# alxfox/AR_Voxel_Project

Hardware: AMD Instinct MI355X
Metric: Mvoxel-views/s (voxels x views / s) + carve wall-time, 512^3 grid x 36 views (higher is better)
Workload: dtype u8; 1 GPU; synthetic sphere silhouettes, 512x512x512 grid, 36 views 640x480, per step: derive bit planes + summed-area tables from the resident u8 masks, then dense carve of a fresh model by all views; one step after the other; views=36, jobs_in_flight=1, parallelism=single GPU, collective=none, cull=True

## Files before the change

### ar_voxel_project_amd/capi.py

```python
from __future__ import annotations

import ctypes as C
import os
from typing import Optional, Sequence, Tuple

import numpy as np

_HERE = os.path.dirname(os.path.abspath(__file__))
LIB_PATH = os.environ.get("ARVX_LIB_PATH") or os.path.join(_HERE, "lib", "libarvx.so")

OCC = 1
SEEN = 2
CARVE_NO_CULL = 1
CARVE_STATS = 2
CARVE_FUSED = 8
CARVE_STREAM = 16
CARVE_FILTER = 64
CARVE_NO_STREAM = 32
CARVE_DENSE_CLASSIFY = 128
CARVE_WHOLE_ITEMS = 256
PATH_DENSE_CLASSIFY = 1
PATH_ITEM_SHARING = 2
PATH_FRESH = 4
PATH_LAZY_CODES = 8
PATH_FUSED = 16
PATH_BRUTE_FORCE = 32
PATH_STREAM = 64
FLOOD_PREPASS = 1
FLOOD_FRESH = 2
VOTES_COUNTS = 1
VOTES_NO_CULL = 2
COMPONENTS_LARGEST = 1
_EXTRA_CARVE_FLAGS = int(os.environ.get("ARVX_CARVE_EXTRA_FLAGS", "0"))
COLOR_CLOSEST = 0
COLOR_AVERAGE = 1

SYMBOLS = [
    "arvx_version", "arvx_last_error", "arvx_device_count", "arvx_projection_assoc",
    "arvx_ctx_create_slab_halo",
    "arvx_set_projection_assoc", "arvx_ctx_set_projection_assoc", "arvx_ctx_projection_assoc",
    "arvx_selftest_project", "arvx_selftest_depth", "arvx_selftest_view_tables",
    "arvx_ctx_create", "arvx_ctx_create_slab", "arvx_ctx_create_striped", "arvx_ctx_destroy",
    "arvx_ctx_set_stream", "arvx_ctx_set_exchange_stream", "arvx_ctx_synchronize", "arvx_ctx_voxels",
    "arvx_compose_projection", "arvx_set_views", "arvx_set_views_device",
    "arvx_set_images", "arvx_state_reset", "arvx_state_upload",
    "arvx_state_download", "arvx_state_device_ptr", "arvx_state_upload_halo",
    "arvx_state_upload_planes", "arvx_state_download_planes", "arvx_state_packet_geometry",
    "arvx_state_download_packets", "arvx_host_register",
    "arvx_host_unregister", "arvx_handle_unseen", "arvx_undistort", "arvx_undistort_device",
    "arvx_pack_occupancy", "arvx_pack_occupancy_global", "arvx_carve", "arvx_carve_views", "arvx_fast_carve",
    "arvx_color", "arvx_surface_count", "arvx_surface_download",
    "arvx_surface_depth_download", "arvx_color_samples",
    "arvx_color_visible", "arvx_surface_visible_download", "arvx_view_depth_download",
    "arvx_photo_carve", "arvx_carve_votes", "arvx_votes_download",
    "arvx_components", "arvx_components_download", "arvx_components_labels_download",
    "arvx_components_keep",
    "arvx_colors_upload", "arvx_closure", "arvx_closure_count", "arvx_closure_download",
    "arvx_closure_download32",
    "arvx_mc_cells", "arvx_mc_cells_download", "arvx_mc_mesh", "arvx_mc_mesh_download",
    "arvx_mc_mesh_download_faces", "arvx_mc_mesh_welded", "arvx_mc_mesh_welded_download",
    "arvx_mc_mesh_smooth", "arvx_mc_mesh_smooth_download",
    "arvx_render", "arvx_render_view", "arvx_render_download", "arvx_render_agreement",
    "arvx_occupancy_packet_words", "arvx_occupancy_compress", "arvx_occupancy_expand",
    "arvx_occupancy_expand_striped", "arvx_occupancy_pack_compress", "arvx_occupancy_expand_striped_others",
    "arvx_export_model", "arvx_get_stats", "arvx_last_carve_path", "arvx_last_fast_carve_path",
    "arvx_selftest_divide",
    "arvx_selftest_round",
]


class ArvxError(RuntimeError):
    def __init__(self, code: int, msg: str):
        super().__init__(f"arvx error {code}: {msg}")
        self.code = code


class Stats(C.Structure):
    _fields_ = [
        ("subtiles", C.c_uint64),
        ("subtiles_carved", C.c_uint64),
        ("subtile_views_mixed", C.c_uint64),
        ("subtile_views_total", C.c_uint64),
        ("surface_voxels", C.c_uint64),
        ("reserved", C.c_uint64 * 3),
        ("host_total_fallbacks", C.c_uint64),
    ]


_libs: dict = {}
ASSOC_RIGHT, ASSOC_LEFT = 0, 1
# ... 55 lines not shown
    lib.arvx_pack_occupancy_global.argtypes = [p, p]
    lib.arvx_carve.argtypes = [p, C.c_uint]
    lib.arvx_carve_views.argtypes = [p, C.c_int, C.c_int, C.c_uint]
    lib.arvx_fast_carve.argtypes = [p]
    lib.arvx_color.argtypes = [p, C.c_int]
    lib.arvx_surface_count.argtypes = [p, C.POINTER(C.c_int64)]
    lib.arvx_surface_download.argtypes = [p, C.POINTER(C.c_int64), f32p]
    lib.arvx_surface_depth_download.argtypes = [p, f32p]
    lib.arvx_colors_upload.argtypes = [p, C.c_int64, C.POINTER(C.c_int64), f32p]
    lib.arvx_closure.argtypes = [p, C.c_int, C.c_int]
    lib.arvx_closure_count.argtypes = [p, C.POINTER(C.c_int64)]
    lib.arvx_closure_download.argtypes = [p, C.POINTER(C.c_int64), f32p]
    lib.arvx_export_model.argtypes = [p, f32p, C.c_int]
    lib.arvx_get_stats.argtypes = [p, C.POINTER(Stats)]
    if hasattr(lib, "arvx_last_carve_path"):
        lib.arvx_last_carve_path.argtypes = [p, C.POINTER(C.c_uint32)]
    if hasattr(lib, "arvx_last_fast_carve_path"):
        lib.arvx_last_fast_carve_path.argtypes = [p, C.POINTER(C.c_uint32)]
    ab_build = bool(os.environ.get("ARVX_LIB_PATH"))
    if hasattr(lib, "arvx_selftest_divide") or not ab_build:
        lib.arvx_selftest_divide.argtypes = [p, C.c_int64, f32p, f32p, f32p, f32p]
    if hasattr(lib, "arvx_selftest_round") or not ab_build:
        lib.arvx_selftest_round.argtypes = [p, C.POINTER(C.c_int64)]
    if hasattr(lib, "arvx_mc_cells") or not ab_build:
        lib.arvx_mc_cells.argtypes = [p, C.POINTER(C.c_int64)]
        lib.arvx_mc_cells_download.argtypes = [p, C.POINTER(C.c_int32)]
    if hasattr(lib, "arvx_occupancy_compress") or not ab_build:
        lib.arvx_occupancy_packet_words.argtypes = [C.c_int64, C.c_int64]
        lib.arvx_occupancy_compress.argtypes = [p, C.c_void_p, C.c_int64, C.c_void_p, C.c_int64]
        lib.arvx_occupancy_expand.argtypes = [p, C.c_void_p, C.c_int, C.c_int, C.c_int64,
                                              C.c_int64, C.c_void_p, C.c_void_p]
        if hasattr(lib, "arvx_occupancy_expand_striped") or not ab_build:
            lib.arvx_occupancy_expand_striped.argtypes = [p, C.c_void_p, C.c_int, C.c_int64,
                                                          C.c_int64, C.c_int64, C.c_void_p,
                                                          C.c_void_p]
        if hasattr(lib, "arvx_occupancy_pack_compress"):
            lib.arvx_occupancy_pack_compress.argtypes = [p, C.c_void_p, C.c_int64, C.c_void_p]
            lib.arvx_occupancy_expand_striped_others.argtypes = [p, C.c_void_p, C.c_int, C.c_int, C.c_int64,
                                                                 C.c_int64, C.c_int64, C.c_void_p, C.c_void_p]
    if hasattr(lib, "arvx_mc_mesh_smooth"):
        lib.arvx_mc_mesh_smooth.argtypes = [p, C.c_int, C.c_float, C.c_float]
        lib.arvx_mc_mesh_smooth_download.argtypes = [p, C.c_void_p, C.c_void_p]
    if hasattr(lib, "arvx_color_visible"):
        lib.arvx_color_visible.argtypes = [p, C.c_int, C.c_float]
        lib.arvx_surface_visible_download.argtypes = [p, C.POINTER(C.c_int32)]
        lib.arvx_view_depth_download.argtypes = [p, C.c_int, f32p]
# ... 576 lines not shown

    def mc_mesh_count(self, apply_unseen: bool = False) -> int:
        n = C.c_int64()
        self._lib.arvx_mc_mesh.argtypes = [C.c_void_p, C.c_int, C.POINTER(C.c_int64)]
        self._ck(self._lib.arvx_mc_mesh(self._h, int(apply_unseen), C.byref(n)))
        return int(n.value)

    def export_model(self, apply_unseen: bool = False) -> np.ndarray:
        out = np.empty((self.nvox, 4), np.float32)
        self._ck(self._lib.arvx_export_model(self._h, _fp(out), int(apply_unseen)))
        return out

    def selftest_divide(self, a0, a1, b) -> np.ndarray:
        a0, a1, b = _f32(a0).reshape(-1), _f32(a1).reshape(-1), _f32(b).reshape(-1)
        out = np.empty((len(b), 4), np.float32)
        self._ck(self._lib.arvx_selftest_divide(self._h, len(b), _fp(a0), _fp(a1), _fp(b), _fp(out)))
        return out

    def selftest_round(self) -> int:
        n = C.c_int64(-1)
        self._ck(self._lib.arvx_selftest_round(self._h, C.byref(n)))
        return int(n.value)

    def stats(self) -> dict:
        s = Stats()
        self._ck(self._lib.arvx_get_stats(self._h, C.byref(s)))
        out = {k: int(getattr(s, k)) for k, _ in Stats._fields_ if k != "reserved"}
        out["slices_evaluated"] = int(s.reserved[0])
        out["open_voxels_in_slices"] = int(s.reserved[1])
        out["mixed_pairs_uniform"] = int(s.reserved[2])
        out["host_total_fallbacks"] = int(s.host_total_fallbacks)
        return out
```

### ar_voxel_project_amd/csrc/arvx_capi.hip

```cpp
#include "arvx/arvx.h"

#include <hip/hip_runtime.h>

#include <cmath>
#include <cstdarg>
#include <cstdio>
#include <cstdlib>
#include <atomic>
#include <cstring>
#include <mutex>
#include <new>
#include <string>
#include <type_traits>
#include <utility>
#include <vector>

#include "arvx_ctx.h"
#include "carve_kernels.h"
#ifdef ARVX_EXPERIMENTS
#include "carve_stream_kernels.h"
#endif
#include "views_kernels.h"
#include "state_kernels.h"
#include "undistort_kernels.h"
#include "color_kernels.h"
#include "closure_kernels.h"
#include "bitplane_kernels.h"
#include "fast_carve_kernels.h"
#include "mc_kernels.h"
#include "mc_mesh_kernels.h"
#include "mc_weld_kernels.h"
#include "mc_smooth_kernels.h"
#include "visibility_kernels.h"
#include "photo_kernels.h"
#include "components_kernels.h"
#include "vote_kernels.h"
#include "render_kernels.h"
#include "exchange_kernels.h"
#include <algorithm>

namespace {
// ... 513 lines not shown
        ctx->pool_images.release();
    }
    ctx->images_ready = false;
    ctx->V = V;
    ctx->W = W;
    ctx->H = H;
    ctx->bgWords = (int)(((((size_t)W * H + 31) / 32 + 1) + 31) / 32 * 32);
    ctx->satW = (W + 1 + 63) / 64 * 64;
    ctx->satH = H + 1;
    ctx->satStride = ctx->satW * ctx->satH;
    if (!same) {
        hipError_t e = ctx->pool_M.reserve((size_t)V * 12 * sizeof(float));
        if (e == hipSuccess) e = ctx->pool_campos.reserve((size_t)V * 3 * sizeof(float));
        if (e == hipSuccess) e = ctx->pool_bg.reserve((size_t)V * ctx->bgWords * sizeof(uint32_t));
        if (e == hipSuccess) e = ctx->pool_sat.reserve((size_t)V * ctx->satStride * sizeof(uint16_t));
        if (e != hipSuccess) {
            ctx->free_views();
            return arvx::fail_hip(e, "hipMalloc(views)", __FILE__, __LINE__);
        }
    }
    const bool same_M = same && ctx->h_M.size() == (size_t)V * 12 &&
                        memcmp(ctx->h_M.data(), M, (size_t)V * 12 * sizeof(float)) == 0;
    if (!same_M) {
        ctx->h_M.assign(M, M + (size_t)V * 12);
        ARVX_HIP(hipMemcpyAsync(ctx->M(), ctx->h_M.data(), (size_t)V * 12 * sizeof(float),
                                hipMemcpyHostToDevice, ctx->stream));
    }
    ctx->has_campos = campos != nullptr;
    if (campos) {
        const bool same_c = same && ctx->h_campos.size() == (size_t)V * 3 &&
                            memcmp(ctx->h_campos.data(), campos, (size_t)V * 3 * sizeof(float)) == 0;
        if (!same_c) {
            ctx->h_campos.assign(campos, campos + (size_t)V * 3);
            ARVX_HIP(hipMemcpyAsync(ctx->campos(), ctx->h_campos.data(),
                                    (size_t)V * 3 * sizeof(float), hipMemcpyHostToDevice,
                                    ctx->stream));
        }
    } else {
        ctx->h_campos.clear();
    }
    return ARVX_OK;
}

static int views_preprocess(Ctx *ctx, const uint8_t *d_masks, int C) {
    const int npix = ctx->W * ctx->H;
    ARVX_HIP(hipGetLastError());
// ... 743 lines not shown
    p.coarseCarved = (uint8_t *)ctx->pool_ccode.p;
    p.cstate = (uint8_t *)ctx->pool_cstate.p;
    p.flags |= 128u;
    ctx->cstate_tiles = 0;
#ifdef ARVX_TIMELINE
    if (int rc = timeline(ctx, (size_t)G * 4, 128, p)) return rc;
#endif
    const bool left = ctx->assoc == ARVX_ASSOC_LEFT, one = p.nchunks == 1;
    if (left && one)
        hipLaunchKernelGGL((arvx::carve_stream_kernel<true, 1>), dim3(G), dim3(256), 0, ctx->stream, p);
    else if (left)
        hipLaunchKernelGGL((arvx::carve_stream_kernel<true, arvx::kMaxChunks>), dim3(G), dim3(256), 0, ctx->stream, p);
    else if (one)
        hipLaunchKernelGGL((arvx::carve_stream_kernel<false, 1>), dim3(G), dim3(256), 0, ctx->stream, p);
    else
        hipLaunchKernelGGL((arvx::carve_stream_kernel<false, arvx::kMaxChunks>), dim3(G), dim3(256), 0, ctx->stream, p);
    ARVX_HIP(hipGetLastError());
    ctx->form = Form::Lazy;
    ctx->cstate_tiles = ncoarse;
    ctx->path_bits = ARVX_PATH_STREAM | ARVX_PATH_FRESH | ARVX_PATH_LAZY_CODES;
    return ARVX_OK;
}
#endif

static int launch_carve(Ctx *ctx, uint16_t *rec, int first, int count, unsigned flags,
                        bool fresh, uint8_t *foreign_code = nullptr) {
    arvx::CarveParams p;
    carve_geometry(ctx, p);
    p.rec = rec;
    carve_views(ctx, p);
    p.stats = ctx->stats();
    p.v0 = first;
    p.v1 = first + count;
    p.flags = (flags & 3u) | (fresh ? 4u : 0u);
    p.ccode = nullptr;
    p.cstate = nullptr;
    p.nchunks = (count + 63) / 64;
    if (flags & ARVX_CARVE_STATS) ARVX_HIP(hipMemsetAsync(ctx->stats(), 0, 64, ctx->stream));
    const size_t rows8 = ((size_t)p.tilesY * p.tilesZ + 7) / 8 * 8;
    const unsigned grid = (unsigned)(rows8 * p.tilesX);
    const bool cull = !(flags & ARVX_CARVE_NO_CULL);
    const bool split = cull && !(flags & ARVX_CARVE_FUSED) && p.nchunks <= arvx::kMaxChunks;
    static const bool two_launches = experiment_flag("ARVX_COARSE_SPLIT");
    const size_t ncoarse = (size_t)p.coarseX * p.coarseY * p.coarseZ;
    if (ctx->ncu <= 0) {
        ctx->ncu = 256;
// ... 95 lines not shown
        (size_t)p.X * p.Y * p.Z <= ((size_t)1 << (split_log2 > 0 ? split_log2 : 26)))
        p.flags |= 8u;
    static const bool force_split = experiment_flag("ARVX_FORCE_SPLIT2");
    if (blocks && force_split) p.flags |= 8u | 64u;
    static const bool no_block_tests = experiment_flag("ARVX_NO_BLOCK_TESTS");
    if (no_block_tests) p.flags |= 32u;
    if (split) {
        if (lazy) {
        } else if (two_launches)
            hipLaunchKernelGGL(arvx::carve_fill_kernel, dim3((unsigned)ncoarse), dim3(256), 0,
                               ctx->stream, p);
        else
            hipLaunchKernelGGL(arvx::carve_coarse_fill_kernel, dim3((unsigned)ncoarse), dim3(256),
                               0, ctx->stream, p);
        ARVX_HIP(hipGetLastError());
        static const int cgrid_env = experiment_int("ARVX_CLASSIFY_WGS");
        const unsigned cgrid = cgrid_env > 0 ? (unsigned)cgrid_env : (unsigned)ncu * 8u;
#ifndef ARVX_CLASSIFY_SPARSE
        const bool dense = !(flags & ARVX_CARVE_STATS) &&
                           ((flags & ARVX_CARVE_DENSE_CLASSIFY) || (size_t)p.X * p.Y * p.Z >= ((size_t)1 << 26));
#else
        const bool dense = false;
#endif
        if (dense)
            hipLaunchKernelGGL(arvx::carve_classify_dense_kernel, dim3((unsigned)ncu * (unsigned)ARVX_DENSE_WGS_PER_CU), dim3(256),
                               0, ctx->stream, p);
        else
            hipLaunchKernelGGL(arvx::carve_classify_kernel, dim3(cgrid), dim3(256), 0, ctx->stream, p);
        ARVX_HIP(hipGetLastError());
        const unsigned pgrid = (unsigned)(p.nwaves / 4);
#ifdef ARVX_TIMELINE
        if (int rc = timeline(ctx, (size_t)pgrid * 4, 64, p)) return rc;
#endif
        const bool left = ctx->assoc == ARVX_ASSOC_LEFT;
        const bool may_split = p.flags & 8u;
#ifdef ARVX_EXPERIMENTS
        const bool filter = (flags & ARVX_CARVE_FILTER) != 0;
        if (blocks && filter && left && may_split)
            hipLaunchKernelGGL((arvx::carve_exact_blocks_kernel<true, true, false, true>), dim3(pgrid), dim3(256), 0,
                               ctx->stream, p);
        else if (blocks && filter && left && fresh)
            hipLaunchKernelGGL((arvx::carve_exact_blocks_kernel<true, false, true, true>), dim3(pgrid), dim3(256), 0,
                               ctx->stream, p);
        else if (blocks && filter && left)
            hipLaunchKernelGGL((arvx::carve_exact_blocks_kernel<true, false, false, true>), dim3(pgrid), dim3(256), 0,
                               ctx->stream, p);
        else if (blocks && filter && may_split)
            hipLaunchKernelGGL((arvx::carve_exact_blocks_kernel<false, true, false, true>), dim3(pgrid), dim3(256), 0,
                               ctx->stream, p);
        else if (blocks && filter && fresh)
            hipLaunchKernelGGL((arvx::carve_exact_blocks_kernel<false, false, true, true>), dim3(pgrid), dim3(256), 0,
                               ctx->stream, p);
        else if (blocks && filter)
            hipLaunchKernelGGL((arvx::carve_exact_blocks_kernel<false, false, false, true>), dim3(pgrid), dim3(256), 0,
                               ctx->stream, p);
        else
#endif
        if (blocks && left && may_split)
            hipLaunchKernelGGL((arvx::carve_exact_blocks_kernel<true, true>), dim3(pgrid), dim3(256), 0,
                               ctx->stream, p);
        else if (blocks && left && fresh)
            hipLaunchKernelGGL((arvx::carve_exact_blocks_kernel<true, false, true>), dim3(pgrid), dim3(256), 0,
                               ctx->stream, p);
        else if (blocks && left)
            hipLaunchKernelGGL((arvx::carve_exact_blocks_kernel<true, false>), dim3(pgrid), dim3(256), 0,
                               ctx->stream, p);
        else if (blocks && may_split)
            hipLaunchKernelGGL((arvx::carve_exact_blocks_kernel<false, true>), dim3(pgrid), dim3(256), 0,
                               ctx->stream, p);
        else if (blocks && fresh)
            hipLaunchKernelGGL((arvx::carve_exact_blocks_kernel<false, false, true>), dim3(pgrid), dim3(256), 0,
                               ctx->stream, p);
        else if (blocks)
            hipLaunchKernelGGL((arvx::carve_exact_blocks_kernel<false, false>), dim3(pgrid), dim3(256), 0,
                               ctx->stream, p);
        else if (left)
            hipLaunchKernelGGL(arvx::carve_exact_kernel<true>, dim3(pgrid), dim3(256), 0,
                               ctx->stream, p);
        else
            hipLaunchKernelGGL(arvx::carve_exact_kernel<false>, dim3(pgrid), dim3(256), 0,
                               ctx->stream, p);
        ARVX_HIP(hipGetLastError());
        ctx->carve_layout = layout_when_done;
        ++ctx->carve_seq;
        ctx->path_bits = (dense ? ARVX_PATH_DENSE_CLASSIFY : 0u) | (may_split ? ARVX_PATH_ITEM_SHARING : 0u) |
                         (fresh ? ARVX_PATH_FRESH : 0u) | (lazy ? ARVX_PATH_LAZY_CODES : 0u);
        ctx->path_dense_grid = dense ? (unsigned)ncu * (unsigned)ARVX_DENSE_WGS_PER_CU : 0u;
        ctx->path_off_listed = (size_t)((uint8_t *)p.undecidedCount - (uint8_t *)ctx->pool_coarse.p);
        ctx->path_off_work = (size_t)((uint8_t *)p.workCount - (uint8_t *)ctx->pool_coarse.p);
        if (lazy && rec == ctx->rec()) ctx->form = Form::Lazy;
        if (p.cstate) ctx->cstate_tiles = ncoarse;
        return ARVX_OK;
    }
#ifdef ARVX_TIMELINE
    if (int rc = timeline(ctx, grid, 32, p)) return rc;
#endif
    if (ctx->assoc == ARVX_ASSOC_LEFT)
        hipLaunchKernelGGL(arvx::carve_fused_kernel<true>, dim3(grid), dim3(256), 0, ctx->stream, p);
    else
        hipLaunchKernelGGL(arvx::carve_fused_kernel<false>, dim3(grid), dim3(256), 0, ctx->stream, p);
    ARVX_HIP(hipGetLastError());
    ctx->path_bits = (cull ? ARVX_PATH_FUSED : ARVX_PATH_BRUTE_FORCE) | (fresh ? ARVX_PATH_FRESH : 0u);
    return ARVX_OK;
}

int arvx_carve_views(arvx_ctx *ctx, int first, int count, unsigned flags) {
    ARVX_CHECK_CTX(ctx);
    if (!ctx->views_ready) return fail(ARVX_ERR_STATE, "arvx_set_views has not been called");
    if (first < 0 || count < 0 || first + count > ctx->V)
        return fail(ARVX_ERR_INVALID, "view range [%d,%d) outside [0,%d)", first, first + count,
                    ctx->V);
    if (count == 0) return ARVX_OK;
#ifndef ARVX_EXPERIMENTS
    if (flags & ARVX_CARVE_STREAM)
        return fail(ARVX_ERR_INVALID, "ARVX_CARVE_STREAM: the one-launch carve is only in -DARVX_EXPERIMENTS "
                                      "builds (libarvx_experiments.so)");
    if (flags & ARVX_CARVE_FILTER)
        return fail(ARVX_ERR_INVALID, "ARVX_CARVE_FILTER: the fp32 projection filter is only in "
                                      "-DARVX_EXPERIMENTS builds (libarvx_experiments.so)");
#endif
    ctx->drop(Event::Carve);
    const bool fresh = ctx->form == Form::Fresh;
    if (fresh) {
        if (int rc = ensure_records(ctx, ctx->pool_rec)) return rc;
    } else if (int rc = need_rec(ctx)) {
// ... 896 lines not shown
}

int arvx_selftest_round(arvx_ctx *ctx, int64_t *mismatches) {
    ARVX_CHECK_CTX(ctx);
    if (!mismatches) return fail(ARVX_ERR_INVALID, "null mismatches");
    *mismatches = -1;
    ARVX_HIP(ctx->pool_scratch.reserve(64));
    unsigned long long *d_bad = (unsigned long long *)ctx->pool_scratch.p;
    ARVX_HIP(hipMemsetAsync(d_bad, 0, sizeof *d_bad, ctx->stream));
    const unsigned ranges[2][2] = {{0x00000000u, 0x4B800000u}, {0x80000000u, 0xBEFFFFFFu}};
    for (const auto &r : ranges) {
        const unsigned long long n = (unsigned long long)r[1] - r[0] + 1;
        hipLaunchKernelGGL(arvx::selftest_round_kernel, dim3((unsigned)((n + 255) / 256)), dim3(256),
                           0, ctx->stream, r[0], r[1], d_bad);
        ARVX_HIP(hipGetLastError());
    }
    unsigned long long bad = 0;
    ARVX_HIP(hipMemcpyAsync(&bad, d_bad, sizeof bad, hipMemcpyDeviceToHost, ctx->stream));
    ARVX_SYNC(ctx);
    *mismatches = (int64_t)bad;
    return ARVX_OK;
}

#ifdef ARVX_TIMELINE
extern "C" int arvx_debug_timeline(arvx_ctx *ctx, unsigned long long *out, int64_t *n) {
    ARVX_CHECK_CTX(ctx);
    *n = ctx->timeline_n;
    if (out && ctx->pool_timeline.p) {
        ARVX_SYNC(ctx);
        ARVX_HIP(hipMemcpy(out, ctx->pool_timeline.p, (size_t)ctx->timeline_n * ctx->timeline_rec,
                           hipMemcpyDeviceToHost));
    }
    return ARVX_OK;
}
#endif


int arvx_colors_upload(arvx_ctx *ctx, int64_t n, const int64_t *index, const float *rgb) {
    ARVX_CHECK_CTX(ctx);
    if (n < 0 || (n > 0 && (!index || !rgb))) return fail(ARVX_ERR_INVALID, "bad colour list");
    ctx->drop(Event::UploadColors);
    std::vector<int> idx((size_t)n);
    const long long own_base = (long long)ctx->X * ctx->Y * (ctx->z0 - ctx->ze0);
    for (int64_t k = 0; k < n; ++k) {
        if (index[k] < 0 || (size_t)index[k] >= ctx->nvox || (k && index[k] <= index[k - 1]))
            return fail(ARVX_ERR_INVALID, "colour indices must be ascending and inside the grid");
// ... 870 lines not shown
```

### ar_voxel_project_amd/csrc/arvx_ctx.h

```cpp
#pragma once

#include <hip/hip_runtime.h>
#include <stdint.h>

#include <vector>

namespace arvx {

int fail_hip(hipError_t e, const char *what, const char *file, int line);
int fail_msg(int code, const char *msg);

#define ARVX_HIP(call)                                                        \
    do {                                                                      \
        hipError_t arvx_e_ = (call);                                          \
        if (arvx_e_ != hipSuccess)                                            \
            return ::arvx::fail_hip(arvx_e_, #call, __FILE__, __LINE__);      \
    } while (0)

struct DevPool {
    enum Size { Headroom, Exact };
    void *p = nullptr;
    size_t cap = 0;
    const bool exact;
    explicit DevPool(Size size = Headroom) : exact(size == Exact) {}
// ... 19 lines not shown
    int device = 0;
    int X = 0, Y = 0, Z = 0;
    int z0 = 0, z1 = 0;
    int ze0 = 0, ze1 = 0;
    int halo = 1;
    int stripe_world = 1, stripe_rank = 0;
    float s = 0.f;
    int assoc = 1;
    size_t nvox = 0;
    size_t nvox_ext = 0;

    unsigned *h_fault = nullptr;
    unsigned *d_fault = nullptr;
    enum Word {
        kSurface, kClosure, kCells, kTris, kVerts,
        kSmoothScan,
        kComponents,
        kDeviceTotals,
        kPhotoRemoved = kDeviceTotals,
        kVisNeed,
        kPacketOcc, kPacketSeen,
        kCompKept, kCompRemoved,
        kRenderNeed, kRenderAgree,
        kWords = kRenderAgree + 3
    };
    static constexpr size_t kHostBlockBytes = 192;
    static_assert(8 + 8 * (size_t)kWords <= kHostBlockBytes, "the count words fit the block");
    long long &word(int w) const { return ((long long *)(h_fault + 2))[w]; }
    long long *word_dev(int w) const { return (long long *)(d_fault + 2) + w; }
    DevPool pool_vstrip;
    size_t vstrip_key = 0;

    DevPool pool_compact;
    DevPool pool_chunk_counts;
    size_t counts_stride = 0;
    int counts_cur = 0;
    bool counts_clean[2] = {false, false};
    unsigned long long compact_tickets = 0;
    uint32_t compact_epoch = 0;
    long long surf_host_count = -1;
    long long clo_host_count = -1;

    hipStream_t own_stream = nullptr;
    hipStream_t stream = nullptr;
    hipStream_t xstream = nullptr;

    enum class Form { Fresh, Records, Lazy };
// ... 31 lines not shown
    DevPool pool_flood_rec{DevPool::Exact};
    DevPool pool_flood_code;
    DevPool pool_coarse{DevPool::Exact};
    DevPool pool_stats{DevPool::Exact};
    unsigned long long *stats() const { return (unsigned long long *)pool_stats.p; }
    unsigned long long host_total_fallbacks = 0;
    DevPool pool_scratch{DevPool::Exact};
    DevPool pool_xscratch;
    DevPool pool_flood{DevPool::Exact};

    bool views_ready = false;
    bool cameras_ready = false;
    bool has_campos = false;
    int V = 0, W = 0, H = 0;
    int bgWords = 0, satStride = 0;
    int satW = 0, satH = 0;
    DevPool pool_M{DevPool::Exact}, pool_campos{DevPool::Exact}, pool_bg{DevPool::Exact},
        pool_sat{DevPool::Exact};
    float *M() const { return (float *)pool_M.p; }
    float *campos() const { return (float *)pool_campos.p; }
    uint32_t *bg() const { return (uint32_t *)pool_bg.p; }
    uint16_t *sat() const { return (uint16_t *)pool_sat.p; }
    std::vector<float> h_M, h_campos;

    DevPool pool_images{DevPool::Exact};
    uint8_t *images() const { return (uint8_t *)pool_images.p; }
    bool images_ready = false;
    int *d_surf_index = nullptr;
    float4 *d_surf_rgba = nullptr;
    float *d_surf_depth = nullptr;
    uint8_t *d_surf_has = nullptr;
    int64_t surf_count = 0;
    std::vector<int> h_surf_index;
    std::vector<uint8_t> h_surf_has;
    bool color_ready = false;
    DevPool pool_col_bits, pool_col_rank;
    bool color_visible = false;
    long long vis_large_need = 0;
    DevPool pool_vis_depth{DevPool::Exact}, pool_vis_large{DevPool::Exact}, pool_vis_views;
    DevPool pool_photo_rm, pool_photo_plane{DevPool::Exact};
    DevPool pool_votes{DevPool::Exact};
    bool votes_ready = false;

    DevPool pool_comp_label{DevPool::Exact}, pool_comp_planes{DevPool::Exact}, pool_comp_rank{DevPool::Exact},
        pool_comp_table, pool_comp_ctl;
    bool comp_ready = false;
// ... 76 lines not shown
        pool_render_large{DevPool::Exact};
    int render_W = 0, render_H = 0;
    bool render_ready = false;
    long long render_need = 0;
    uint8_t *h_render_bg = nullptr;
    size_t render_bg_cap = 0;
    hipEvent_t render_bg_done = nullptr;

    ~Ctx() {
        if (render_bg_done) (void)hipEventDestroy(render_bg_done);
        if (h_render_bg) (void)hipHostFree(h_render_bg);
        if (h_fault) (void)hipHostFree(h_fault);
    }
    void free_mc() {
        d_mc_cells = nullptr;
        mc_count = 0;
        mc_ready = false;
    }
    void free_views() {
        pool_M.release();
        pool_campos.release();
        pool_bg.release();
        pool_sat.release();
        views_ready = false;
        cameras_ready = false;
    }
};

}

struct arvx_ctx : arvx::Ctx {};
```

### ar_voxel_project_amd/csrc/arvx_device.h

```cpp
#pragma once

#include <hip/hip_runtime.h>
#include <stdint.h>

namespace arvx {

constexpr int kTileX = 64, kTileY = 8, kTileZ = 8;
constexpr int kSubX = 16;
constexpr int kCoarseX = 64;
constexpr uint32_t kDone4 = 0x02020202u;
constexpr int kMaxImageDim = 16384;
constexpr int kWorkLists = 64;
constexpr int kPoolCounters = 8;
constexpr int kCounterStride = 64;
constexpr int kMaxChunks = 4;

enum : int { kClsOut = 0, kClsFg = 1, kClsCarved = 2, kClsMixed = 3, kFastDiv = 4 };

constexpr int kRecU16 = 128;

struct CarveParams {
    uint16_t *rec;
    const uint8_t *ccode;
    const float *M;
// ... 16 lines not shown
    unsigned long long *coarseMixed;
    unsigned long long *coarseFg;
    uint8_t *coarseCarved;
    int coarsePerWg;
    uint8_t *cstate;
    int *undecidedList;
    int *undecidedCount;
    int *undecidedCountNext;
    int *workCount;
    int *poolNext;
    int nwaves;
    int workCap;
    unsigned long long *itemInfo;
    unsigned long long *itemMasks;
    int *sctl;
    unsigned long long *listG;
    unsigned long long *itemG;
    unsigned epoch;
    int listCap;
    int listStride, itemStride;
    int nA, cwA;
    int splitLog2;
    unsigned *fault;
};

__device__ __forceinline__ int global_z(const CarveParams &p, int lz) {
    return p.zoff + (((lz >> 3) * p.zstride + p.zphase) << 3) + (lz & 7);
}

__host__ __device__ __forceinline__ size_t rec_index(const CarveParams &p, int tx, int ty, int tz,
                                                     int wave) {
    const int ct = tx + p.coarseX * ((ty >> p.cyShift) + p.coarseY * (tz >> p.czShift));
    const int tl = (ty & ((1 << p.cyShift) - 1)) | ((tz & ((1 << p.czShift) - 1)) << p.cyShift);
    return ((((size_t)ct << (p.cyShift + p.czShift)) + tl) << 2) + wave;
}
__host__ __device__ __forceinline__ size_t rec_count(const CarveParams &p) {
    return ((size_t)p.coarseX * p.coarseY * p.coarseZ) << (p.cyShift + p.czShift + 2);
}
__device__ __forceinline__ int coarse_of(const CarveParams &p, int tx, int ty, int tz) {
    return tx + p.coarseX * ((ty >> p.cyShift) + p.coarseY * (tz >> p.czShift));
}
constexpr int kCodeWritten = 0x80;
__device__ __forceinline__ int lazy_code(const CarveParams &p, int tx, int ty, int tz) {
    if (!p.ccode) return 0;
    const int c = (int)p.ccode[coarse_of(p, tx, ty, tz)];
    return (c & kCodeWritten) ? 0 : c;
// ... 98 lines not shown
```

### ar_voxel_project_amd/csrc/carve_kernels.h

```cpp
#pragma once

#include "arvx_device.h"

namespace arvx {

struct BoxW {
    float wy0, wy1, wx0, wx1, wz0, wz1;
};

__device__ __forceinline__ BoxW make_box(float s, int x0, int x1, int y0, int y1, int z0, int z1) {
    BoxW b;
    b.wy0 = (float)y0 * s;
    b.wy1 = (float)y1 * s;
    b.wx0 = (float)x0 * s;
    b.wx1 = (float)x1 * s;
    b.wz0 = (float)(-z0) * s;
    b.wz1 = (float)(-z1) * s;
    return b;
}

typedef uint16_t sat_t;
struct RectQ {
    int code;
    int fast;
// ... 69 lines not shown
    q.code = -1;
    return q;
}
__device__ __forceinline__ int rect_finish(const RectQ &q, int s00, int s01, int s10, int s11) {
    const int cnt = (s11 - s01 - s10 + s00) & 0xffff;
    if (cnt == 0) return kClsCarved;
    return (cnt == q.dx * q.dy) ? kClsFg : (kClsMixed | q.fast);
}
__device__ inline int classify_box_m(const float (&M)[12], const BoxW b, int W, int H,
                                     const sat_t *__restrict__ sat, int satW) {
    const RectQ q = rect_prepare(M, b, W, H, satW);
    if (q.code >= 0) return q.code;
    const sat_t *e = sat + q.base;
    return rect_finish(q, e[0], e[q.dx], e[q.dy * satW], e[q.dy * satW + q.dx]);
}
__device__ inline int classify_box(const float *__restrict__ M, const BoxW b, int W, int H,
                                   const sat_t *__restrict__ sat, int satW) {
    float Mr[12];
#pragma unroll
    for (int i = 0; i < 12; ++i) Mr[i] = M[i];
    return classify_box_m(Mr, b, W, H, sat, satW);
}

__device__ __forceinline__ void coarse_reset_counters(const CarveParams &p) {
    if (blockIdx.x == 0 && p.workCount)
        for (int i = threadIdx.x; i < (kWorkLists + kPoolCounters) * kCounterStride; i += blockDim.x)
            p.workCount[i] = 0;
    if (blockIdx.x == 0 && threadIdx.x == 0 && p.undecidedCountNext) *p.undecidedCountNext = 0;
}

__device__ __forceinline__ int coarse_classify(const CarveParams &p, const int ct, const int lane) {
    const int cx = ct % p.coarseX;
    const int cy = (ct / p.coarseX) % p.coarseY;
    const int cz = ct / (p.coarseX * p.coarseY);
    const int cyN = 8 << p.cyShift, czN = 8 << p.czShift;
    const int x0 = cx * kCoarseX, y0 = cy * cyN, z0 = cz * czN;
    const BoxW box = make_box(p.s, x0, min(x0 + kCoarseX - 1, p.X - 1), y0,
                              min(y0 + cyN - 1, p.Y - 1), global_z(p, z0),
                              global_z(p, min(z0 + czN - 1, p.Z - 1)));
    bool any_carved = false, any_mixed = false, any_fg = false;
    int chunk = 0;
    for (int vc = p.v0; vc < p.v1; vc += 64, ++chunk) {
        const int myv = vc + lane;
        int cls = kClsOut;
        if (myv < p.v1)
            cls = classify_box(p.M + 12 * myv, box, p.W, p.H, p.sat + (size_t)myv * p.satStride,
// ... 1230 lines not shown
        if (!n) break;
        const int myb = q == 0 ? vb[0] : (q == 1 ? vb[1] : (q == 2 ? vb[2] : vb[3]));
        int cls = kClsOut;
        if (q < n && inside) {
            const int view = vbase + myb;
            cls = classify_box(p.M + 12 * view, box, p.W, p.H, p.sat + (size_t)view * p.satStride,
                               p.satW) & 3;
        }
        const unsigned long long c = __ballot(cls == kClsCarved), f = __ballot(cls == kClsFg),
                                 x = __ballot(cls == kClsMixed);
        carved |= (unsigned)((c | (c >> 16) | (c >> 32) | (c >> 48)) & 0xffffu);
        seen |= (unsigned)((f | (f >> 16) | (f >> 32) | (f >> 48)) & 0xffffu);
#pragma unroll
        for (int k = 0; k < 4; ++k)
            if (k < n) {
                const unsigned need16 = (unsigned)((x >> (16 * k)) & 0xffffu);
                if (lane == slot) needLanes = need16;
                ++slot;
            }
    }
    return needLanes;
}

template <int NB>
__device__ __forceinline__ unsigned block_tests_lds(const CarveParams &p, const float *sM,
                                                    const SubTile &t, int vrel,
                                                    unsigned long long views, int lane,
                                                    unsigned &carved, unsigned &seen) {
    const int blk = lane & 15, q = lane >> 4;
    const int j = blk & 3, m = blk >> 2, byi = m >> 1, bzi = m & 1;
    const int x0 = t.sx0 + 4 * j, y0 = t.sy0 + 4 * byi, z0 = t.sz0 + 4 * bzi;
    const bool inside = x0 < p.X && y0 < p.Y && z0 < p.Z;
    const BoxW box = make_box(p.s, x0, min(x0 + 3, p.X - 1), y0, min(y0 + 3, p.Y - 1),
                              global_z(p, z0), global_z(p, min(z0 + 3, p.Z - 1)));
    unsigned needLanes = 0;
    int slot = 0;
    while (views) {
        RectQ rq[NB];
        int nv[NB], myv[NB];
        int s00[NB], s01[NB], s10[NB], s11[NB];
#pragma unroll
        for (int g = 0; g < NB; ++g) {
            int vb[4];
            nv[g] = 0;
#pragma unroll
            for (int k = 0; k < 4; ++k) {
// ... 31 lines not shown
                (rq[g].code >= 0 ? rq[g].code : rect_finish(rq[g], s00[g], s01[g], s10[g], s11[g])) & 3;
            const unsigned long long c = __ballot(cls == kClsCarved), f = __ballot(cls == kClsFg),
                                     x = __ballot(cls == kClsMixed);
            carved |= (unsigned)((c | (c >> 16) | (c >> 32) | (c >> 48)) & 0xffffu);
            seen |= (unsigned)((f | (f >> 16) | (f >> 32) | (f >> 48)) & 0xffffu);
#pragma unroll
            for (int k = 0; k < 4; ++k)
                if (k < nv[g]) {
                    const unsigned need16 = (unsigned)((x >> (16 * k)) & 0xffffu);
                    if (lane == slot) needLanes = need16;
                    ++slot;
                }
        }
    }
    return needLanes;
}

#ifndef ARVX_EXACT_WAVES_PER_SIMD
#define ARVX_EXACT_WAVES_PER_SIMD 4
#endif
#ifndef ARVX_EXACT_SPLIT_WAVES_PER_SIMD
#define ARVX_EXACT_SPLIT_WAVES_PER_SIMD 3
#endif
template <bool LEFT, bool SPLIT = true, bool FRESH = false, bool FILTER = false>
__global__ __launch_bounds__(256, (SPLIT && !FRESH ? ARVX_EXACT_SPLIT_WAVES_PER_SIMD : ARVX_EXACT_WAVES_PER_SIMD))
void carve_exact_blocks_kernel(const CarveParams p) {
#ifdef ARVX_TIMELINE
    WaveTimeline wave_timeline(p.timeline);
#endif
    const int lane = threadIdx.x & 63;
    const int lx = lane & 3, ly = (lane >> 2) & 3, lz = lane >> 4;
    for_each_work_item<SPLIT>(p, lane, blockIdx.x * 4 + (threadIdx.x >> 6), p.nwaves,
                          [&](const size_t it, const int part, const int list, const int pshift_) {
            const int pshift = SPLIT ? pshift_ : 0;
#ifndef ARVX_NO_SETPRIO
            switch (list >> 4) {
                case 0: __builtin_amdgcn_s_setprio(3); break;
                case 1: __builtin_amdgcn_s_setprio(2); break;
                case 2: __builtin_amdgcn_s_setprio(1); break;
                default: __builtin_amdgcn_s_setprio(0); break;
            }
#endif
            const unsigned long long info = p.itemInfo[it];
            unsigned long long mixed0 = p.itemMasks[it * p.nchunks * 2];
            unsigned long long fast0 = p.itemMasks[it * p.nchunks * 2 + 1];
#ifdef ARVX_TIMELINE
            { volatile unsigned long long sink = info; (void)sink; }
// ... 38 lines not shown
            }
            float wmax[3] = {0.f, 0.f, 0.f};
            if (FILTER) {
                wmax[0] = (float)(t.sy0 + 7) * p.s;
                wmax[1] = (float)(t.sx0 + 15) * p.s;
                wmax[2] = fmaxf(fabsf((float)(-global_z(p, t.sz0)) * p.s),
                                fabsf((float)(-global_z(p, t.sz0 + 7)) * p.s));
            }
            bool done = false;
#ifdef ARVX_TIMELINE
            wave_timeline.tick(1);
#endif
            for (int c = 0; c < p.nchunks && !done; ++c) {
                unsigned long long mixed =
                    uniform64(c ? p.itemMasks[(it * p.nchunks + c) * 2] : mixed0);
                const unsigned long long fastdiv =
                    uniform64(c ? p.itemMasks[(it * p.nchunks + c) * 2 + 1] : fast0);
                unsigned bcarved = 0, bseen = 0;
#ifdef ARVX_EXPERIMENTS
                const bool no_bt = p.flags & 32u;
#else
                constexpr bool no_bt = false;
#endif
                const unsigned needLanes = no_bt
                                               ? 0xffffu
                                               : block_tests(p, t, p.v0 + 64 * c, mixed, part, pshift,
                                                             lane, bcarved, bseen);
#pragma unroll
                for (int m = 0; m < 4; ++m) {
                    uint32_t w = st[m];
#pragma unroll
                    for (int j = 0; j < 4; ++j) {
                        if ((bseen >> (4 * m + j)) & 1u) w |= 2u << (8 * j);
                        if ((bcarved >> (4 * m + j)) & 1u)
                            w = (w & ~(0xffu << (8 * j))) | (2u << (8 * j));
                    }
                    st[m] = w;
                }
                done = __all(st[0] == kDone4 && st[1] == kDone4 && st[2] == kDone4 &&
                             st[3] == kDone4);
                int slot = 0;
                for (int nth = 0; mixed && !done; ++nth) {
                    const int b = __ffsll((long long)mixed) - 1;
                    mixed &= mixed - 1;
                    if ((nth & ((1 << pshift) - 1)) != part) continue;
                    const unsigned need = no_bt
                                              ? 0xffffu
                                              : (unsigned)__builtin_amdgcn_readlane(needLanes, slot);
                    ++slot;
                    if (!need) continue;
// ... 125 lines not shown
```

### include/arvx/arvx.h

```cpp
#ifndef ARVX_H
#define ARVX_H

#include <stddef.h>
#include <stdint.h>

#ifdef __cplusplus
extern "C" {
#endif

#define ARVX_VERSION 100

enum {
    ARVX_OK = 0,
    ARVX_ERR_INVALID = 1,
    ARVX_ERR_HIP = 2,
    ARVX_ERR_STATE = 3,
    ARVX_ERR_NOMEM = 4
};

#define ARVX_OCC 1u
#define ARVX_SEEN 2u

#define ARVX_CARVE_NO_CULL 1u
#define ARVX_CARVE_STATS 2u
// ... 141 lines not shown
int arvx_mc_mesh_welded(arvx_ctx *ctx, int apply_unseen, int64_t *vertices, int64_t *triangles);
int arvx_mc_mesh_welded_download(arvx_ctx *ctx, float *verts, uint32_t *faces, float *vertex_rgb);

int arvx_mc_mesh_smooth(arvx_ctx *ctx, int iterations, float lambda, float mu);
int arvx_mc_mesh_smooth_download(arvx_ctx *ctx, float *verts, float *normals);

int arvx_render(arvx_ctx *ctx, const float M[12], int W, int H, const uint8_t *background,
                size_t bg_stride);
int arvx_render_view(arvx_ctx *ctx, int view);
int arvx_render_download(arvx_ctx *ctx, uint8_t *bgr, float *depth, int32_t *id);
int arvx_render_agreement(arvx_ctx *ctx, int view, int64_t counts[3]);

int arvx_export_model(arvx_ctx *ctx, float *rgba, int apply_unseen);

int arvx_get_stats(arvx_ctx *ctx, arvx_stats *out);

#define ARVX_PATH_DENSE_CLASSIFY 1u
#define ARVX_PATH_ITEM_SHARING 2u
#define ARVX_PATH_FRESH 4u
#define ARVX_PATH_LAZY_CODES 8u
#define ARVX_PATH_FUSED 16u
#define ARVX_PATH_BRUTE_FORCE 32u
#define ARVX_PATH_STREAM 64u
int arvx_last_carve_path(arvx_ctx *ctx, uint32_t out[4]);

#define ARVX_FLOOD_PREPASS 1u
#define ARVX_FLOOD_FRESH 2u
int arvx_last_fast_carve_path(arvx_ctx *ctx, uint32_t out[4]);

int arvx_selftest_divide(arvx_ctx *ctx, int64_t n, const float *a0, const float *a1,
                         const float *b, float *out);

int arvx_selftest_project(arvx_ctx *ctx, int64_t n, const float M[12], float voxel_size,
                          const int32_t *xyz, float *rows_uv);
int arvx_selftest_depth(arvx_ctx *ctx, int64_t n, const float campos[3], float voxel_size,
                        const int32_t *xyz, float *depth);

int arvx_selftest_view_tables(arvx_ctx *ctx, int view, uint32_t *bg_bits, uint16_t *table, int *ld);

int arvx_selftest_round(arvx_ctx *ctx, int64_t *mismatches);

#ifdef __cplusplus
}
#endif
#endif
```

Before: 50.17 million Mvoxel-views/s.

## Cache per-view block projection rectangles for the fresh dense carve path

Adds a device table that stores, for every 4x4x4 block and view, its projected summed-area-table rectangle (origin and extents) or a trivial out/mixed code. The table depends only on the camera matrices and grid geometry. It is built once after two consecutive eligible carves and invalidated when the matrices change. The exact-blocks carve kernel gets a cached variant that reads these entries instead of projecting each block's corners, which removes per-block projection arithmetic. In exchange it reads several hundred MB of table per step, pays a one-time build with a host sync, and only covers the non-split fresh path.

```diff
diff --git a/ar_voxel_project_amd/capi.py b/ar_voxel_project_amd/capi.py
--- a/ar_voxel_project_amd/capi.py
+++ b/ar_voxel_project_amd/capi.py
@@ -26,6 +26,7 @@
 PATH_FUSED = 16
 PATH_BRUTE_FORCE = 32
 PATH_STREAM = 64
+PATH_RECT_BLOCKS = 128
 FLOOD_PREPASS = 1
 FLOOD_FRESH = 2
 VOTES_COUNTS = 1
@@ -66,6 +67,7 @@
     "arvx_export_model", "arvx_get_stats", "arvx_last_carve_path", "arvx_last_fast_carve_path",
     "arvx_selftest_divide",
     "arvx_selftest_round",
+    "arvx_ctx_set_rect_cache_limit", "arvx_selftest_rect_cache",
 ]
 
 
@@ -167,6 +169,9 @@
         lib.arvx_selftest_divide.argtypes = [p, C.c_int64, f32p, f32p, f32p, f32p]
     if hasattr(lib, "arvx_selftest_round") or not ab_build:
         lib.arvx_selftest_round.argtypes = [p, C.POINTER(C.c_int64)]
+    if hasattr(lib, "arvx_selftest_rect_cache") or not ab_build:
+        lib.arvx_ctx_set_rect_cache_limit.argtypes = [p, C.c_uint64]
+        lib.arvx_selftest_rect_cache.argtypes = [p, C.POINTER(C.c_int64)]
     if hasattr(lib, "arvx_mc_cells") or not ab_build:
         lib.arvx_mc_cells.argtypes = [p, C.POINTER(C.c_int64)]
         lib.arvx_mc_cells_download.argtypes = [p, C.POINTER(C.c_int32)]
@@ -789,6 +794,14 @@
         self._ck(self._lib.arvx_selftest_round(self._h, C.byref(n)))
         return int(n.value)
 
+    def set_rect_cache_limit(self, nbytes: int) -> None:
+        self._ck(self._lib.arvx_ctx_set_rect_cache_limit(self._h, nbytes))
+
+    def selftest_rect_cache(self) -> int:
+        n = C.c_int64(-2)
+        self._ck(self._lib.arvx_selftest_rect_cache(self._h, C.byref(n)))
+        return int(n.value)
+
     def stats(self) -> dict:
         s = Stats()
         self._ck(self._lib.arvx_get_stats(self._h, C.byref(s)))
diff --git a/ar_voxel_project_amd/csrc/arvx_capi.hip b/ar_voxel_project_amd/csrc/arvx_capi.hip
--- a/ar_voxel_project_amd/csrc/arvx_capi.hip
+++ b/ar_voxel_project_amd/csrc/arvx_capi.hip
@@ -17,6 +17,7 @@
 
 #include "arvx_ctx.h"
 #include "carve_kernels.h"
+#include "rect_cache_kernels.h"
 #ifdef ARVX_EXPERIMENTS
 #include "carve_stream_kernels.h"
 #endif
@@ -576,6 +577,7 @@
     const bool same_M = same && ctx->h_M.size() == (size_t)V * 12 &&
                         memcmp(ctx->h_M.data(), M, (size_t)V * 12 * sizeof(float)) == 0;
     if (!same_M) {
+        ctx->rect_invalidate();
         ctx->h_M.assign(M, M + (size_t)V * 12);
         ARVX_HIP(hipMemcpyAsync(ctx->M(), ctx->h_M.data(), (size_t)V * 12 * sizeof(float),
                                 hipMemcpyHostToDevice, ctx->stream));
@@ -1365,6 +1367,54 @@
     return ARVX_OK;
 }
 #endif
+
+
+static arvx::RectBits rect_bits(const Ctx *ctx) {
+    arvx::RectBits rb = {1, 1, 0};
+    while ((1 << rb.xb) < ctx->W) ++rb.xb;
+    while ((1 << rb.yb) < ctx->H) ++rb.yb;
+    rb.db = (32 - rb.xb - rb.yb) / 2;
+    return rb;
+}
+static size_t rect_entries(const Ctx *ctx, const arvx::CarveParams &p) {
+    return (arvx::rec_count(p) << 4) * (size_t)ctx->V;
+}
+static void rect_params(const Ctx *ctx, arvx::CarveParams &p) {
+    const arvx::RectBits rb = rect_bits(ctx);
+    p.rcXB = rb.xb;
+    p.rcYB = rb.yb;
+    p.rcDB = rb.db;
+}
+
+static int rect_cache_prepare(Ctx *ctx, arvx::CarveParams &p) {
+    if (!ctx->rect_limit) return ARVX_OK;
+    if (ctx->rect_streak < 2) ++ctx->rect_streak;
+    if (ctx->rect_streak < 2) return ARVX_OK;
+    rect_params(ctx, p);
+    if (ctx->rect_state == Ctx::Rect::None) {
+        ctx->rect_state = Ctx::Rect::Refused;
+        const size_t n = rect_entries(ctx, p), bytes = n * sizeof(uint32_t);
+        if (p.rcDB < 1 || bytes > ctx->rect_limit) return ARVX_OK;
+        if (ctx->pool_rect.reserve(bytes) != hipSuccess) {
+            (void)hipGetLastError();
+            return ARVX_OK;
+        }
+        ctx->word(Ctx::kRectMiss) = 0;
+        hipLaunchKernelGGL(arvx::rect_cache_block_kernel<false>, dim3((unsigned)std::min<size_t>((n + 255) / 256, 65536)),
+                           dim3(256), 0, ctx->stream, p, (uint32_t *)ctx->pool_rect.p, n,
+                           ctx->word_dev(Ctx::kRectMiss), (unsigned long long *)nullptr);
+        ARVX_HIP(hipGetLastError());
+        ARVX_SYNC(ctx);
+        if (ctx->word(Ctx::kRectMiss)) {
+            ctx->word(Ctx::kRectMiss) = 0;
+            ctx->pool_rect.release();
+            return ARVX_OK;
+        }
+        ctx->rect_state = Ctx::Rect::Built;
+    }
+    if (ctx->rect_state == Ctx::Rect::Built) p.rcBlk = (const uint32_t *)ctx->pool_rect.p;
+    return ARVX_OK;
+}
 
 static int launch_carve(Ctx *ctx, uint16_t *rec, int first, int count, unsigned flags,
                         bool fresh, uint8_t *foreign_code = nullptr) {
@@ -1506,6 +1556,11 @@
 #else
         const bool dense = false;
 #endif
+        if (dense && blocks && fresh && !(p.flags & 8u) && rec == ctx->rec()) {
+            if (int rc = rect_cache_prepare(ctx, p)) return rc;
+        } else {
+            ctx->rect_streak = 0;
+        }
         if (dense)
             hipLaunchKernelGGL(arvx::carve_classify_dense_kernel, dim3((unsigned)ncu * (unsigned)ARVX_DENSE_WGS_PER_CU), dim3(256),
                                0, ctx->stream, p);
@@ -1518,7 +1573,9 @@
 #endif
         const bool left = ctx->assoc == ARVX_ASSOC_LEFT;
         const bool may_split = p.flags & 8u;
+        bool cached = blocks && fresh && !may_split && p.rcBlk;
 #ifdef ARVX_EXPERIMENTS
+        if (flags & ARVX_CARVE_FILTER) cached = false;
         const bool filter = (flags & ARVX_CARVE_FILTER) != 0;
         if (blocks && filter && left && may_split)
             hipLaunchKernelGGL((arvx::carve_exact_blocks_kernel<true, true, false, true>), dim3(pgrid), dim3(256), 0,
@@ -1540,7 +1597,13 @@
                                ctx->stream, p);
         else
 #endif
-        if (blocks && left && may_split)
+        if (cached && left)
+            hipLaunchKernelGGL((arvx::carve_exact_blocks_kernel<true, false, true, false, true>), dim3(pgrid), dim3(256), 0,
+                               ctx->stream, p);
+        else if (cached)
+            hipLaunchKernelGGL((arvx::carve_exact_blocks_kernel<false, false, true, false, true>), dim3(pgrid), dim3(256), 0,
+                               ctx->stream, p);
+        else if (blocks && left && may_split)
             hipLaunchKernelGGL((arvx::carve_exact_blocks_kernel<true, true>), dim3(pgrid), dim3(256), 0,
                                ctx->stream, p);
         else if (blocks && left && fresh)
@@ -1568,7 +1631,8 @@
         ctx->carve_layout = layout_when_done;
         ++ctx->carve_seq;
         ctx->path_bits = (dense ? ARVX_PATH_DENSE_CLASSIFY : 0u) | (may_split ? ARVX_PATH_ITEM_SHARING : 0u) |
-                         (fresh ? ARVX_PATH_FRESH : 0u) | (lazy ? ARVX_PATH_LAZY_CODES : 0u);
+                         (fresh ? ARVX_PATH_FRESH : 0u) | (lazy ? ARVX_PATH_LAZY_CODES : 0u) |
+                         (cached ? ARVX_PATH_RECT_BLOCKS : 0u);
         ctx->path_dense_grid = dense ? (unsigned)ncu * (unsigned)ARVX_DENSE_WGS_PER_CU : 0u;
         ctx->path_off_listed = (size_t)((uint8_t *)p.undecidedCount - (uint8_t *)ctx->pool_coarse.p);
         ctx->path_off_work = (size_t)((uint8_t *)p.workCount - (uint8_t *)ctx->pool_coarse.p);
@@ -1585,6 +1649,7 @@
         hipLaunchKernelGGL(arvx::carve_fused_kernel<false>, dim3(grid), dim3(256), 0, ctx->stream, p);
     ARVX_HIP(hipGetLastError());
     ctx->path_bits = (cull ? ARVX_PATH_FUSED : ARVX_PATH_BRUTE_FORCE) | (fresh ? ARVX_PATH_FRESH : 0u);
+    ctx->rect_streak = 0;
     return ARVX_OK;
 }
 
@@ -2527,6 +2592,40 @@
     return ARVX_OK;
 }
 
+int arvx_ctx_set_rect_cache_limit(arvx_ctx *ctx, uint64_t bytes) {
+    ARVX_CHECK_CTX(ctx);
+    if (bytes > (uint64_t)1 << 46) return fail(ARVX_ERR_INVALID, "limit of %llu bytes", (unsigned long long)bytes);
+    if (ctx->pool_rect.p) ARVX_SYNC(ctx);
+    ctx->pool_rect.release();
+    ctx->rect_state = Ctx::Rect::None;
+    ctx->rect_limit = (size_t)bytes;
+    return ARVX_OK;
+}
+
+int arvx_selftest_rect_cache(arvx_ctx *ctx, int64_t *mismatches) {
+    ARVX_CHECK_CTX(ctx);
+    if (!mismatches) return fail(ARVX_ERR_INVALID, "null mismatches");
+    *mismatches = -1;
+    if (ctx->rect_state != Ctx::Rect::Built) return ARVX_OK;
+    arvx::CarveParams p;
+    carve_geometry(ctx, p);
+    carve_views(ctx, p);
+    rect_params(ctx, p);
+    ARVX_HIP(ctx->pool_scratch.reserve(64));
+    unsigned long long *d_bad = (unsigned long long *)ctx->pool_scratch.p;
+    ARVX_HIP(hipMemsetAsync(d_bad, 0, sizeof *d_bad, ctx->stream));
+    const size_t n = rect_entries(ctx, p);
+    hipLaunchKernelGGL(arvx::rect_cache_block_kernel<true>, dim3((unsigned)std::min<size_t>((n + 255) / 256, 65536)),
+                       dim3(256), 0, ctx->stream, p, (uint32_t *)ctx->pool_rect.p, n, (long long *)nullptr,
+                       d_bad);
+    ARVX_HIP(hipGetLastError());
+    unsigned long long bad = 0;
+    ARVX_HIP(hipMemcpyAsync(&bad, d_bad, sizeof bad, hipMemcpyDeviceToHost, ctx->stream));
+    ARVX_SYNC(ctx);
+    *mismatches = (int64_t)bad;
+    return ARVX_OK;
+}
+
 #ifdef ARVX_TIMELINE
 extern "C" int arvx_debug_timeline(arvx_ctx *ctx, unsigned long long *out, int64_t *n) {
     ARVX_CHECK_CTX(ctx);
diff --git a/ar_voxel_project_amd/csrc/arvx_ctx.h b/ar_voxel_project_amd/csrc/arvx_ctx.h
--- a/ar_voxel_project_amd/csrc/arvx_ctx.h
+++ b/ar_voxel_project_amd/csrc/arvx_ctx.h
@@ -65,7 +65,8 @@
         kPacketOcc, kPacketSeen,
         kCompKept, kCompRemoved,
         kRenderNeed, kRenderAgree,
-        kWords = kRenderAgree + 3
+        kRectMiss = kRenderAgree + 3,
+        kWords
     };
     static constexpr size_t kHostBlockBytes = 192;
     static_assert(8 + 8 * (size_t)kWords <= kHostBlockBytes, "the count words fit the block");
@@ -143,6 +144,15 @@
     uint32_t *bg() const { return (uint32_t *)pool_bg.p; }
     uint16_t *sat() const { return (uint16_t *)pool_sat.p; }
     std::vector<float> h_M, h_campos;
+    enum class Rect { None, Built, Refused };
+    Rect rect_state = Rect::None;
+    int rect_streak = 0;
+    size_t rect_limit = (size_t)1 << 30;
+    DevPool pool_rect{DevPool::Exact};
+    void rect_invalidate() {
+        rect_state = Rect::None;
+        rect_streak = 0;
+    }
 
     DevPool pool_images{DevPool::Exact};
     uint8_t *images() const { return (uint8_t *)pool_images.p; }
@@ -265,6 +275,8 @@
         pool_campos.release();
         pool_bg.release();
         pool_sat.release();
+        pool_rect.release();
+        rect_invalidate();
         views_ready = false;
         cameras_ready = false;
     }
diff --git a/ar_voxel_project_amd/csrc/arvx_device.h b/ar_voxel_project_amd/csrc/arvx_device.h
--- a/ar_voxel_project_amd/csrc/arvx_device.h
+++ b/ar_voxel_project_amd/csrc/arvx_device.h
@@ -62,6 +62,8 @@
     int nA, cwA;
     int splitLog2;
     unsigned *fault;
+    const uint32_t *rcBlk;
+    int rcXB, rcYB, rcDB;
 };
 
 __device__ __forceinline__ int global_z(const CarveParams &p, int lz) {
diff --git a/ar_voxel_project_amd/csrc/carve_kernels.h b/ar_voxel_project_amd/csrc/carve_kernels.h
--- a/ar_voxel_project_amd/csrc/carve_kernels.h
+++ b/ar_voxel_project_amd/csrc/carve_kernels.h
@@ -115,6 +115,34 @@
     return classify_box_m(Mr, b, W, H, sat, satW);
 }
 
+struct RectBits {
+    int xb, yb, db;
+};
+constexpr uint32_t kRectBlkOut = 0u, kRectBlkMixed = 1u;
+__device__ __forceinline__ bool rect_pack_block(const RectQ &q, int satW, const RectBits rb, uint32_t &e) {
+    e = kRectBlkMixed;
+    if (q.code >= 0) {
+        e = (q.code & 3) == kClsOut ? kRectBlkOut : kRectBlkMixed;
+        return true;
+    }
+    if (q.dx >= (1 << rb.db) || q.dy >= (1 << rb.db)) return false;
+    const int pylo = q.base / satW, pxlo = q.base - pylo * satW;
+    e = (uint32_t)pxlo | ((uint32_t)pylo << rb.xb) | ((uint32_t)q.dx << (rb.xb + rb.yb)) |
+        ((uint32_t)q.dy << (rb.xb + rb.yb + rb.db));
+    return true;
+}
+__device__ __forceinline__ int classify_block_entry(const uint32_t e, const RectBits rb,
+                                                    const sat_t *__restrict__ sat, int satW) {
+    if (!(e >> (rb.xb + rb.yb))) return e == kRectBlkOut ? kClsOut : kClsMixed;
+    const int pxlo = (int)__builtin_amdgcn_ubfe(e, 0u, (unsigned)rb.xb);
+    const int pylo = (int)__builtin_amdgcn_ubfe(e, (unsigned)rb.xb, (unsigned)rb.yb);
+    RectQ q;
+    q.fast = 0;
+    q.dx = (int)__builtin_amdgcn_ubfe(e, (unsigned)(rb.xb + rb.yb), (unsigned)rb.db);
+    q.dy = (int)(e >> (rb.xb + rb.yb + rb.db));
+    const sat_t *s = sat + (pylo * satW + pxlo);
+    return rect_finish(q, s[0], s[q.dx], s[q.dy * satW], s[q.dy * satW + q.dx]);
+}
 __device__ __forceinline__ void coarse_reset_counters(const CarveParams &p) {
     if (blockIdx.x == 0 && p.workCount)
         for (int i = threadIdx.x; i < (kWorkLists + kPoolCounters) * kCounterStride; i += blockDim.x)
@@ -1391,6 +1419,49 @@
     return needLanes;
 }
 
+__device__ __forceinline__ unsigned block_tests_cached(const CarveParams &p, const size_t ri, int vbase,
+                                                       unsigned long long views, int lane,
+                                                       unsigned &carved, unsigned &seen) {
+    const int q = lane >> 4;
+    const RectBits rb = {p.rcXB, p.rcYB, p.rcDB};
+    const size_t vstride = rec_count(p) << 4;
+    const uint32_t *const tab = p.rcBlk + ((ri << 4) + (lane & 15));
+    unsigned needLanes = 0;
+    int slot = 0;
+    while (views) {
+        int vb[4];
+        int n = 0;
+#pragma unroll
+        for (int k = 0; k < 4; ++k) {
+            vb[k] = 0;
+            if (views) {
+                vb[k] = __ffsll((long long)views) - 1;
+                views &= views - 1;
+                n = k + 1;
+            }
+        }
+        const int myb = q == 0 ? vb[0] : (q == 1 ? vb[1] : (q == 2 ? vb[2] : vb[3]));
+        int cls = kClsOut;
+        if (q < n) {
+            const int view = vbase + myb;
+            cls = classify_block_entry(tab[(size_t)view * vstride], rb,
+                                       p.sat + (size_t)view * p.satStride, p.satW) & 3;
+        }
+        const unsigned long long c = __ballot(cls == kClsCarved), f = __ballot(cls == kClsFg),
+                                 x = __ballot(cls == kClsMixed);
+        carved |= (unsigned)((c | (c >> 16) | (c >> 32) | (c >> 48)) & 0xffffu);
+        seen |= (unsigned)((f | (f >> 16) | (f >> 32) | (f >> 48)) & 0xffffu);
+#pragma unroll
+        for (int k = 0; k < 4; ++k)
+            if (k < n) {
+                const unsigned need16 = (unsigned)((x >> (16 * k)) & 0xffffu);
+                if (lane == slot) needLanes = need16;
+                ++slot;
+            }
+    }
+    return needLanes;
+}
+
 template <int NB>
 __device__ __forceinline__ unsigned block_tests_lds(const CarveParams &p, const float *sM,
                                                     const SubTile &t, int vrel,
@@ -1468,7 +1539,7 @@
 #ifndef ARVX_EXACT_SPLIT_WAVES_PER_SIMD
 #define ARVX_EXACT_SPLIT_WAVES_PER_SIMD 3
 #endif
-template <bool LEFT, bool SPLIT = true, bool FRESH = false, bool FILTER = false>
+template <bool LEFT, bool SPLIT = true, bool FRESH = false, bool FILTER = false, bool CACHED = false>
 __global__ __launch_bounds__(256, (SPLIT && !FRESH ? ARVX_EXACT_SPLIT_WAVES_PER_SIMD : ARVX_EXACT_WAVES_PER_SIMD))
 void carve_exact_blocks_kernel(const CarveParams p) {
 #ifdef ARVX_TIMELINE
@@ -1553,10 +1624,15 @@
 #else
                 constexpr bool no_bt = false;
 #endif
-                const unsigned needLanes = no_bt
-                                               ? 0xffffu
-                                               : block_tests(p, t, p.v0 + 64 * c, mixed, part, pshift,
-                                                             lane, bcarved, bseen);
+                unsigned needLanes = 0xffffu;
+                if constexpr (CACHED) {
+                    static_assert(!SPLIT, "the table's variant takes every view of an item");
+                    if (!no_bt)
+                        needLanes = block_tests_cached(p, rec_index(p, tx, ty, tz, wave), p.v0 + 64 * c,
+                                                       mixed, lane, bcarved, bseen);
+                } else if (!no_bt) {
+                    needLanes = block_tests(p, t, p.v0 + 64 * c, mixed, part, pshift, lane, bcarved, bseen);
+                }
 #pragma unroll
                 for (int m = 0; m < 4; ++m) {
                     uint32_t w = st[m];
diff --git a/ar_voxel_project_amd/csrc/rect_cache_kernels.h b/ar_voxel_project_amd/csrc/rect_cache_kernels.h
--- /dev/null
+++ b/ar_voxel_project_amd/csrc/rect_cache_kernels.h
@@ -0,0 +1,53 @@
+#pragma once
+
+#include "carve_kernels.h"
+
+namespace arvx {
+
+__device__ inline bool rect_cache_block_entry(const CarveParams &p, int view, size_t ri, int blk,
+                                              uint32_t &e) {
+    const int tshift = p.cyShift + p.czShift;
+    const int wave = (int)(ri & 3);
+    const int tl = (int)((ri >> 2) & ((1u << tshift) - 1u));
+    const int ct = (int)(ri >> (tshift + 2));
+    const int tx = ct % p.coarseX;
+    const int ty = (((ct / p.coarseX) % p.coarseY) << p.cyShift) + (tl & ((1 << p.cyShift) - 1));
+    const int tz = ((ct / (p.coarseX * p.coarseY)) << p.czShift) + (tl >> p.cyShift);
+    const int sx0 = tx * kTileX + wave * kSubX, sy0 = ty * kTileY, sz0 = tz * kTileZ;
+    const int j = blk & 3, m = blk >> 2, byi = m >> 1, bzi = m & 1;
+    const int x0 = sx0 + 4 * j, y0 = sy0 + 4 * byi, z0 = sz0 + 4 * bzi;
+    RectQ q;
+    q.code = kClsOut;
+    q.fast = q.base = q.dx = q.dy = 0;
+    if (x0 < p.X && y0 < p.Y && z0 < p.Z) {
+        const BoxW box = make_box(p.s, x0, min(x0 + 3, p.X - 1), y0, min(y0 + 3, p.Y - 1),
+                                  global_z(p, z0), global_z(p, min(z0 + 3, p.Z - 1)));
+        float Mr[12];
+#pragma unroll
+        for (int i = 0; i < 12; ++i) Mr[i] = p.M[12 * view + i];
+        q = rect_prepare(Mr, box, p.W, p.H, p.satW);
+    }
+    const RectBits rb = {p.rcXB, p.rcYB, p.rcDB};
+    return rect_pack_block(q, p.satW, rb, e);
+}
+
+template <bool CHECK>
+__global__ __launch_bounds__(256) void rect_cache_block_kernel(const CarveParams p, uint32_t *__restrict__ blk,
+                                                               size_t nblk, long long *miss,
+                                                               unsigned long long *bad) {
+    const size_t per_view = rec_count(p) << 4;
+    const size_t stride = (size_t)gridDim.x * blockDim.x;
+    for (size_t i = (size_t)blockIdx.x * blockDim.x + threadIdx.x; i < nblk; i += stride) {
+        const size_t in_view = i % per_view;
+        uint32_t e;
+        const bool fits = rect_cache_block_entry(p, (int)(i / per_view), in_view >> 4, (int)(in_view & 15), e);
+        if (CHECK) {
+            if (!fits || blk[i] != e) atomicAdd(bad, 1ull);
+        } else {
+            blk[i] = e;
+            if (!fits) *miss = 1;
+        }
+    }
+}
+
+}
diff --git a/include/arvx/arvx.h b/include/arvx/arvx.h
--- a/include/arvx/arvx.h
+++ b/include/arvx/arvx.h
@@ -187,6 +187,7 @@
 #define ARVX_PATH_FUSED 16u
 #define ARVX_PATH_BRUTE_FORCE 32u
 #define ARVX_PATH_STREAM 64u
+#define ARVX_PATH_RECT_BLOCKS 128u
 int arvx_last_carve_path(arvx_ctx *ctx, uint32_t out[4]);
 
 #define ARVX_FLOOD_PREPASS 1u
@@ -205,6 +206,10 @@
 
 int arvx_selftest_round(arvx_ctx *ctx, int64_t *mismatches);
 
+int arvx_ctx_set_rect_cache_limit(arvx_ctx *ctx, uint64_t bytes);
+
+int arvx_selftest_rect_cache(arvx_ctx *ctx, int64_t *mismatches);
+
 #ifdef __cplusplus
 }
 #endif
```

Measured after the change: 52.73 million Mvoxel-views/s (median of 6 runs). +5.1%, better.
